# mkofinas/aether

Measured on AMD Instinct MI355X. Metric: edge-messages/sec (forward, electrostatic N=20 batch=128 per GPU), higher is better.
Workload: dtype f32; 1 GPU; electrostatic-2d-N20-B128; num_dims=2, nodes_per_graph=20, graphs_per_gpu=128, edges_per_gpu=48640, hidden=64, launch=hipgraph (10 steps per replay), parallelism=graphs sharded over 1 rank(s), no forward collective

## Files before the change

aether_amd/csrc/aether_hip.hip:

```cpp

#include <hip/hip_runtime.h>
#include <hipcub/hipcub.hpp>

#include <cstdint>
#include <cstdio>
#include <cstring>

#include "common.h"
#include "streamed.h"
#include "fused.h"
#include "backward.h"
#include "fused_bwd.h"
#include "edge_acc.h"
#include "input_grad.h"
#include "rollout_bwd.h"
#include "wide.h"
#include "seq2seq.h"
#include "s2s_filter.h"
#include "s2s_step.h"
#include "s2s_markov.h"
#include "s2s_charges.h"
#include "s2s_locs.h"
#include "s2s_dnri.h"
#include "dynfield.h"
// ... 1479 lines not shown
    if (!p || !grads || !x || !vel || !charges || !grad_field || !workspace)
        return fail(AETHER_EINVAL, "dynamic_field_backward: null pointer");
    {
        const float* const* gp = reinterpret_cast<const float* const*>(grads);
        for (size_t k = 0; k < sizeof(AetherDynFieldParams) / sizeof(const float*); ++k)
            if (!gp[k]) return fail(AETHER_EINVAL, "dynamic_field_backward: null gradient pointer");
    }
    if (num_dims != 2 && num_dims != 3) return fail(AETHER_EINVAL, "dynamic_field_backward: num_dims must be 2 or 3");
    if (n_graphs <= 0 || nodes_per_graph <= 0 || nodes_per_graph > DYNFIELD_MAX_NODES)
        return fail(AETHER_EINVAL, "dynamic_field_backward: 1..2048 nodes per graph");
    if (n_graphs >= ((int64_t)1 << 31)) return fail(AETHER_EINVAL, "dynamic_field_backward: too many graphs");
    if (workspace_bytes < aether_dynamic_field_backward_workspace_bytes(num_dims, n_graphs))
        return fail(AETHER_ESPACE, "dynamic_field_backward: workspace too small");
    hipStream_t st = (hipStream_t)stream;
    float* partial = reinterpret_cast<float*>(align_up((size_t)workspace, 256));
    if (num_dims == 2) {
        kb_dynfield<2><<<dim3((unsigned)n_graphs), dim3(256), 0, st>>>(*p, x, vel, charges, grad_field, partial, nodes_per_graph,
                                                                       grad_field_inputs);
        k_dynfield_reduce<2><<<dim3((DynOff<2>::total + 31) / 32), dim3(256), 0, st>>>(partial, n_graphs, *grads);
    } else {
        kb_dynfield<3><<<dim3((unsigned)n_graphs), dim3(256), 0, st>>>(*p, x, vel, charges, grad_field, partial, nodes_per_graph,
                                                                       grad_field_inputs);
        k_dynfield_reduce<3><<<dim3((DynOff<3>::total + 31) / 32), dim3(256), 0, st>>>(partial, n_graphs, *grads);
    }
    HIP_OK(hipGetLastError());
    return AETHER_OK;
}

int64_t aether_debug_fetch(const char* name, int num_dims, int64_t n_nodes, int64_t n_edges,
                           const void* workspace, float* dst, void* stream) {
    if (!name || !workspace || !dst) return fail(AETHER_EINVAL, "debug_fetch: null pointer");
    if (num_dims != 2 && num_dims != 3) return fail(AETHER_EINVAL, "debug_fetch: num_dims");
    const int D = num_dims, NIS = D == 2 ? 16 : 24;
    WsLayout W(n_nodes, n_edges, D, false);
    const char* ws = (const char*)workspace;
    hipStream_t st = (hipStream_t)stream;
    auto copy2d = [&](const float* src, int64_t rows, int src_ld, int col0, int cols) -> int64_t {
        hipError_t e = hipMemcpy2DAsync(dst, (size_t)cols * 4, src + col0, (size_t)src_ld * 4,
                                        (size_t)cols * 4, (size_t)rows, hipMemcpyDeviceToDevice, st);
        if (e != hipSuccess) { fail(AETHER_EHIP, hipGetErrorString(e)); return AETHER_EHIP; }
        return rows * cols;
    };
    const float* ni = (const float*)(ws + W.nodeinfo);
    if (!strcmp(name, "field")) return copy2d(ni, n_nodes, NIS, 2 * D, D);
    if (!strcmp(name, "R")) return copy2d(ni, n_nodes, NIS, 3 * D, D * D);
    if (!strcmp(name, "canon")) return copy2d(ni, n_nodes, NIS, 3 * D + D * D, 2 * D);
    if (!strcmp(name, "stamps"))
        return copy2d((const float*)(ws + W.stamps), 4096, FUSED_STAMPS, 0, FUSED_STAMPS);
    if (name[0] == 'x' && name[1] >= '0' && name[1] <= '4' && !name[2])
        return copy2d((const float*)(ws + W.x[name[1] - '0']), n_nodes, H, 0, H);
    if (name[0] == 'e' && name[1] >= '1' && name[1] <= '4' && !name[2])
        return copy2d((const float*)(ws + W.e[name[1] - '1']), n_edges, H, 0, H);
    if (!strcmp(name, "efeat"))
        return copy2d((const float*)(ws + W.feat), n_edges, FPAD, 0, FPAD);
    return fail(AETHER_EINVAL, "debug_fetch: unknown name");
}

int aether_debug_split(const float* x, int n_tiles, uint16_t* hi, uint16_t* lo, int* on, float* scale, float* y) {
    if (!x || !hi || !lo || !on || !scale || !y) return fail(AETHER_EINVAL, "debug_split: null pointer");
    if (n_tiles < 0) return fail(AETHER_EINVAL, "debug_split: n_tiles");
    if (n_tiles == 0) return AETHER_OK;
    k_debug_split<<<dim3(1), dim3(64 * DEBUG_SPLIT_WAVES), 0, nullptr>>>(x, n_tiles, hi, lo, on, scale, y);
    HIP_OK(hipGetLastError());
    return AETHER_OK;
}

int aether_s2s_launch_stats(AetherS2SLaunchStats* stats) {
    if (!stats) return fail(AETHER_EINVAL, "s2s_launch_stats: null pointer");
    *stats = g_s2s_stats;
    return AETHER_OK;
}

void aether_s2s_launch_stats_reset(void) { g_s2s_stats = AetherS2SLaunchStats{}; }

int aether_debug_fused_packed_edge(int wave, int lane) {
    if (wave < 0 || wave >= FUSED_PACK_WAVES || lane < 0 || lane >= FUSED_PACK_LANES) return -1;
    return fused_packed_edge(wave, lane);
}

int aether_debug_fused_wave_role(int what, int wave) {
    if (wave < 0 || wave >= 12) return -1;
    if (what == 0) return wave >= FUSED_FRAME_WAVE0 && fused_frame_tile(wave) < FUSED_MAX_NODES / 16 ? fused_frame_tile(wave) : -1;
    if (what == 1) return wave >= FUSED_X0_WAVE0 && fused_x0_rowblock(wave) < FUSED_X0_WAVES ? fused_x0_rowblock(wave) : -1;
    return -1;
}

#include "host_wide.inc"
#include "host_rollout_train.inc"

}
```

aether_amd/csrc/fused.h:

```cpp
#pragma once
#include "common.h"
#include "fused_layout.h"
#include "fused_graph.h"
#include "fused_handoff.h"

namespace {

struct FusedDebug {
    float* nodeinfo; float* x[5]; float* e[4];
    float* n[4]; float* ps[3]; float* pr[3]; float* feat;
    int* flags;
    int* errword;
    const float* wimg;
    float* stamps;
    StepExtras step;
};
constexpr int FUSED_STAMPS = 512;

#ifdef AETHER_FUSED_STAMPS
#define FUSED_STAMP(id)                                                                          \
    do {                                                                                         \
        if (tid == 0 && blockIdx.x < 4096)                                                       \
            dbg.stamps[blockIdx.x * FUSED_STAMPS + (id)] = (float)(wall_clock64() - t_entry) * 0.01f; \
    } while (0)
// ... 11 lines not shown
    } while (0)
#define FUSED_PSTAMP_W(w_, k_, dep_)                                                              \
    do {                                                                                         \
        asm volatile("v_mov_b32 %0, %0" : "+v"(dep_));                                           \
        if (wave == (w_) && lane == 0 && blockIdx.x < 4096)                                      \
            dbg.stamps[blockIdx.x * FUSED_STAMPS + 400 + (k_)] =                                  \
                (float)(__builtin_amdgcn_s_memtime() - c_entry);                                 \
    } while (0)
#define FUSED_PSTAMP(k_, dep_) FUSED_PSTAMP_W(0, k_, dep_)
#else
#define FUSED_STAMP(id)
#define FUSED_WSTAMP(layer_, r_, k_)
#define FUSED_WSTAMP_ROWS(layer_, r_)
#define FUSED_PSTAMP(k_, dep_)
#define FUSED_PSTAMP_W(w_, k_, dep_)
#endif

template <int D, int NW, int ROUNDS, bool KEEP, bool GRAN = false>
__global__ void __launch_bounds__(NW * 64)
k_fused(AetherParams P, const float* __restrict__ x, const float* __restrict__ vel,
        const float* __restrict__ charges, const float* __restrict__ edge_attr_orig,
        const int32_t* __restrict__ perm, const int32_t* __restrict__ send_s,
        const int32_t* __restrict__ recv_s, const int32_t* __restrict__ rowptr,
        const FusedWG* __restrict__ wgdesc, const uint32_t* __restrict__ trec, const int4* __restrict__ ledge,
        const int32_t* __restrict__ nrange, FusedDebug dbg, float* __restrict__ out) {
    constexpr bool keep = KEEP;
    using NI = NodeInfo<D>;
    using L = FusedLds<NW, ROUNDS>;
    constexpr int THREADS = NW * 64;
    constexpr int FIN = 2 * D + 16;
    static_assert(NW == 8 || NW == 12, "waves 0-7 run the node phase; NW == 12 adds four waves that run step 3 (DESIGN.md 4.1)");
    static_assert(NW == 8 || (ROUNDS == 1 && !KEEP), "the 12-wave kernel owns one tile per wave and saves nothing for the backward");
    static_assert(!GRAN || NW == 12, "granules are the 12-wave kernel's hand-off");
    constexpr bool LATE = NW == 12 || ROUNDS == 2;
    constexpr bool EARLY = NW == 12;
    extern __shared__ __attribute__((aligned(16))) float smem[];
    float* wA = smem + L::WA;
    float* wB = smem + L::WB;
    const float* cblk = smem + L::CBLK;
    float* xbuf = smem + L::XBUF;
    float* nbuf = smem + L::NBUF;
    float* psb = smem + L::PS;
    float* prb = smem + L::PR;
    float* ninfo = smem + L::NINFO;
    float* part = smem + L::PART;

    const int tid = threadIdx.x, lane = tid & 63, wave = tid >> 6;
    const int i = lane & 15, q = lane >> 4;
    const FusedWG wg = wgdesc[blockIdx.x];
    const int vb = wg.vb, nv = wg.ve - wg.vb;
    const int nb = wg.nb, ne = wg.ne;
    const int n = ne - nb, off = nb - vb;
    const int eb = wg.eb, m = wg.m;
    const int n_tiles = (m + 15) >> 4;
    const int na = wg.na;
    typedef __attribute__((address_space(3))) volatile int lds_word;
    lds_word* arrived = (lds_word*)(smem + L::ARRIVED);
    if (tid == 0) { arrived[0] = 0; arrived[1] = 0; }
#ifdef AETHER_FUSED_STAMPS
    const unsigned long long t_entry = wall_clock64();
    const unsigned long long c_entry = __builtin_amdgcn_s_memtime();
#endif
    FUSED_STAMP(0);

    auto dma_images = [&](int layer_) {
        const int na_frag = layer_ == 1 ? 8 : 16, nw_frag = na_frag + 16;
        const int total = nw_frag + FUSED_CBLK / 256;
        const int wv = __builtin_amdgcn_readfirstlane(wave);
        __builtin_assume(wv >= 0 && wv < NW);
        const int g_img = fused_wimg_offset(layer_, 0), g_cb = fused_cblk_offset(layer_);
        const int l_cb = L::CBLK + (layer_ & 1) * FUSED_CBLK;
        constexpr int MAXF = (32 + FUSED_CBLK / 256 + NW - 1) / NW;
#pragma unroll
        for (int j = 0; j < MAXF; ++j) {
            const int f = wv + NW * j;
            if (f < total) {
                const int img = f < na_frag ? f * 256 : FUSED_WIMG + (f - na_frag) * 256;
                const int soff = f < nw_frag ? g_img + img : g_cb + (f - nw_frag) * 256;
                const int doff = f < nw_frag ? L::WA + img : l_cb + (f - nw_frag) * 256;
                __builtin_amdgcn_global_load_lds(dbg.wimg + soff + lane * 4, (__attribute__((address_space(3))) void*)(smem + doff), 16, 0, 0);
            }
        }
    };
    dma_images(1);
    FUSED_STAMP(1);

    constexpr int FR = ROUNDS < 2 ? ROUNDS : 2;
    constexpr bool PACKED = NW == 12;
    constexpr bool FIMG = NW == 12;
    constexpr bool FRAMES = NW == 12;
    f32x4 x0_acc = f32x4{0.f, 0.f, 0.f, 0.f}, x0_ar = f32x4{0.f, 0.f, 0.f, 0.f};
    const int f_local = PACKED ? fused_packed_edge(wave, lane) : 16 * (NW * (lane >> 4) + wave) + (lane & 15);
    const bool f_have = (PACKED ? wave < FUSED_PACK_WAVES && lane < FUSED_PACK_LANES : lane < 16 * FR) && f_local < m;
    int4 f_e = make_int4(0, 0, 0, 0);
    f32x2 f_ea = {0.0f, 0.0f};
    int4 t_e[ROUNDS];
    unsigned seg_ends[ROUNDS];
    unsigned seg_rows[ROUNDS][4];
    {
        const int wv = __builtin_amdgcn_readfirstlane(wave);
#pragma unroll
        for (int r = 0; r < ROUNDS; ++r) {
            const int stile = NW * r + wv;
            const uint32_t* rec = trec + (size_t)(wg.tile0 + (stile < n_tiles ? stile : 0)) * FUSED_TREC;
            seg_ends[r] = stile < n_tiles ? __builtin_amdgcn_readfirstlane(rec[0]) : 0u;
#pragma unroll
            for (int w = 0; w < 4; ++w) seg_rows[r][w] = __builtin_amdgcn_readfirstlane(rec[2 + w]);
        }
    }
    const int aslot = (tid >> 4) & (FUSED_MAX_NODES - 1), ac4 = (tid & 15) * 4;
    int4 nr_rec;
    const int4* own_desc = reinterpret_cast<const int4*>(wgdesc + blockIdx.x);
    const int4* le_base = m > 0 ? ledge + eb : own_desc;
    const int4* nr_base = n > 0 ? reinterpret_cast<const int4*>(nrange) + nb : own_desc;
    const float* ea_base = m > 0 ? edge_attr_orig : reinterpret_cast<const float*>(own_desc);
    const float* qattr = dbg.step.qattr;
    auto index_stage_a = [&]() {
        f_e = le_base[f_have ? f_local : 0];
#pragma unroll
        for (int r = 0; r < ROUNDS; ++r) {
            const int tile = NW * r + wave, local = 16 * tile + i;
            t_e[r] = le_base[local < m ? local : 0];
        }
        nr_rec = nr_base[aslot < n ? aslot : 0];
    };
    auto index_select = [&]() {
        if (!f_have) f_e = make_int4(0, 0, 0, 0);
#pragma unroll
        for (int r = 0; r < ROUNDS; ++r) {
            t_e[r].x = m > 0 ? t_e[r].x : 0; t_e[r].y = m > 0 ? t_e[r].y : vb;
            t_e[r].z = m > 0 ? t_e[r].z : nb; t_e[r].w = m > 0 ? t_e[r].w : 0;
        }
    };
    auto index_stage_b = [&]() -> f32x2 {
        f32x2 v;
        if (qattr) {
            v[0] = qattr[f_e.y]; v[1] = qattr[f_e.z];
        } else {
            const float* ea = ea_base + 2 * (int64_t)f_e.w;
            v[0] = ea[0]; v[1] = ea[1];
        }
        return v;
    };

    {
        const int vtiles = (nv + 15) >> 4;
        if (wave < vtiles) {
            const float* p_ext;
            int node;
            bool live;
            int64_t g;
            float pz[D], vz[D], ef[D];
            float ch;
            float zc[6][3], a1[2][6];
            f32x4 w2f[2][2], w4f[2], acc1[2], acc2[2];
            f32x4 acc3 = f32x4{0.f, 0.f, 0.f, 0.f};
            float ar[4][2];
            f32x4 acc0[4];
            f32x4 fimg[FIMG ? FUSED_FIMG_CHUNKS : 1];
            if constexpr (FIMG) {
                const auto fimg_rsrc = __builtin_amdgcn_make_buffer_rsrc(const_cast<float*>(dbg.wimg) + fused_fimg_offset(), 0, FUSED_FIMG * 4, 0x00020000);
                p_ext = dbg.step.ext_field ? dbg.step.ext_field : x;
                asm volatile("" :: "s"(fimg_rsrc), "s"(p_ext), "s"(x), "s"(vel), "s"(charges), "s"(le_base), "s"(nr_base),
                             "s"(ea_base), "s"(qattr));
                node = 16 * wave + i;
                live = node < nv;
                g = vb + (live ? node : 0);
// ... 374 lines not shown
        arange = (unsigned)at0 | (unsigned)at1 << 8 | (unsigned)bt0 << 16 | (unsigned)bt1 << 24;
        const int deg = (nr.y - nr.x) + (nr.w - nr.z);
        adeg = (float)(deg > 1 ? deg : 1);
    }

    f16x8 wsh[2], wsl[2], wrh[2], wrl[2];
    f16x8 wf_h[4], wf_l[4];
    const auto wimg_rsrc = __builtin_amdgcn_make_buffer_rsrc(const_cast<float*>(dbg.wimg), 0, FUSED_WIMG_SPLIT * 4, 0x00020000);
    const int lane16 = lane * 16;
#pragma unroll 1
    for (int layer = 1; layer <= 4; ++layer) {
        const float* cb = cblk + (layer & 1) * FUSED_CBLK;
        const int mb2 = wave & 7;
        const int mb3 = wave & 3, tn3 = (wave >> 2) & 1;
        const bool act3 = wave < 8;
        const bool one_tile = NW == 12 ? true : n <= 16;
        const int tn4 = one_tile ? 0 : tn3;
        const int tn3s = tn4;
        const bool do3 = NW == 12 ? wave >= 8 : act3 && (one_tile ? wave >= 4 : 16 * tn3 < n);
        const bool do_s = act3 && (one_tile ? wave < 4 : true);
        const bool do_r = act3 && (one_tile ? wave >= 4 : true);
        f16x8 w3h[2], w3l[2], w4h[4], w4l[4];
        auto frag = [&](int block_bytes, int kb) -> f16x8 {
            return __builtin_bit_cast(f16x8, __builtin_amdgcn_raw_buffer_load_b128(wimg_rsrc, lane16, block_bytes + kb * 1024, 0));
        };
        auto load_frags = [&](int which, int mb, int MBN, int KBN, int kb0, int nkb, f16x8* wh, f16x8* wl) {
            if constexpr (ROUNDS == 3 && KEEP) {
                const f16x8* w = reinterpret_cast<const f16x8*>(dbg.wimg + fused_nimg_offset(layer, which)) +
                                 __builtin_amdgcn_readfirstlane(mb) * (KBN * 64);
#pragma unroll
                for (int kb = kb0; kb < kb0 + nkb; ++kb) {
                    wh[kb] = w[kb * 64 + lane];
                    wl[kb] = w[MBN * KBN * 64 + kb * 64 + lane];
                }
                return;
            }
            int lbytes = (layer - 1) * (FUSED_NIMG_LAYER * 4);
            asm volatile("" : "+s"(lbytes));
            const int blk = fused_nimg_offset(1, which) * 4 + lbytes + __builtin_amdgcn_readfirstlane(mb) * (KBN * 1024);
#pragma unroll
            for (int kb = kb0; kb < kb0 + nkb; ++kb) {
                wh[kb] = frag(blk, kb);
                wl[kb] = frag(blk + MBN * KBN * 1024, kb);
            }
        };
        auto issue_loads = [&](int part) {
            if constexpr (NW == 12) {
                const int wv = __builtin_amdgcn_readfirstlane(wave);
                int lbytes = (layer - 1) * (FUSED_NIMG_LAYER * 4);
                asm volatile("" : "+s"(lbytes));
                const bool w4 = wv >= 8;
                const int blk01 = lbytes + (w4 ? fused_nimg_offset(1, 1) * 4 + (wv & 3) * 4096 : fused_nimg_offset(1, 0) * 4 + wv * 2048);
                const int blk23 = w4 ? blk01 + 2048 : lbytes + (wv < 4 ? fused_nimg_offset(1, 2) : fused_nimg_offset(1, 3)) * 4 + (wv & 3) * 2048;
                const int lo23 = w4 ? 16 * 1024 : 8 * 1024;
                if (part == 1) {
#pragma unroll
                    for (int kb = 0; kb < 2; ++kb) {
                        wf_h[kb] = frag(blk01, kb);
                        wf_l[kb] = frag(blk01 + 16 * 1024, kb);
                    }
                }
                if (part == 3) {
#pragma unroll
                    for (int kb = 0; kb < 2; ++kb) {
                        wf_h[2 + kb] = frag(blk23, kb);
                        wf_l[2 + kb] = frag(blk23 + lo23, kb);
                    }
                }
            } else {
            if (part == 1 && act3) load_frags(0, mb2, 8, 2, 0, 2, w3h, w3l);
            if ((part == 2 || part == 3) && do3) load_frags(1, mb3, 4, 4, 2 * (part - 2), 2, w4h, w4l);
            if (part == 4 && (layer < 4 ? true : act3)) {
                if (layer == 4 || do_s) load_frags(2, mb3, 4, 2, 0, 2, wsh, wsl);
                if (layer == 4 || do_r) load_frags(3, mb3, 4, 2, 0, 2, wrh, wrl);
            }
            }
        };
        const bool xch = wg.partner >= 0 && layer > 1;
        auto front_gemm = [&](int r, f32x4 (&acc)[4], bool last, bool late_tile) {
            if (layer == 1) {
#pragma unroll
                for (int mb = 0; mb < 4; ++mb) acc[mb] = ld4(cb + CB_B1 + 16 * mb + 4 * q);
                f32x4 bop[2] = {e[r][0], e[r][1]};
                gemm_split<4, 1>(wA, bop, acc, lane);
            } else {
                f32x4 pr[4], st[4];
#pragma unroll
                for (int mb = 0; mb < 4; ++mb) {
                    pr[mb] = ld4(prb + rl[r] * LDW + 16 * mb + 4 * q);
                    st[mb] = pr[mb] + ld4(psb + sl[r] * LDW + 16 * mb + 4 * q);
                }
                if (late_tile) {
                    const bool late = 16 * (NW * r + wave) + i >= na;
#pragma unroll
                    for (int mb = 0; mb < 4; ++mb)
#pragma unroll
                        for (int c = 0; c < 4; ++c) st[mb][c] = late ? pr[mb][c] : st[mb][c];
                }
                if constexpr (LATE) {
                    if constexpr (EARLY) {
#pragma unroll
                        for (int mb = 0; mb < 4; ++mb) acc[mb] = e[r][mb] + st[mb];
                    } else {
                        f32x4 g[4];
#pragma unroll
                        for (int mb = 0; mb < 4; ++mb) g[mb] = f32x4{0.f, 0.f, 0.f, 0.f};
                        gemm_split<4, 2>(wA, e[r], g, lane);
#pragma unroll
                        for (int mb = 0; mb < 4; ++mb) acc[mb] = g[mb] + st[mb];
                    }
                } else {
#pragma unroll
                    for (int mb = 0; mb < 4; ++mb) acc[mb] = st[mb];
                    gemm_split<4, 2>(wA, e[r], acc, lane);
                }
            }
        };
        auto late_add = [&](int r, f32x4 (&acc)[4]) {
            const bool late = 16 * (NW * r + wave) + i >= na;
            f32x4 ps[4];
#pragma unroll
            for (int mb = 0; mb < 4; ++mb) ps[mb] = ld4(psb + sl[r] * LDW + 16 * mb + 4 * q);
            asm volatile("s_waitcnt lgkmcnt(0)" : "+v"(ps[0]), "+v"(ps[1]), "+v"(ps[2]), "+v"(ps[3]));
#pragma unroll
            for (int mb = 0; mb < 4; ++mb)
#pragma unroll
                for (int c = 0; c < 4; ++c) acc[mb][c] = late ? acc[mb][c] + ps[mb][c] : acc[mb][c];
        };
        auto receive_partner_rows = [&]() {
            if constexpr (GRAN) {
                FUSED_WSTAMP(layer, 0, 6);
                gran_receive(gran_rsrc(dbg.flags, wg.goff, vb, nv), layer, nv, n, off, lane, psb, arrived, dbg.errword);
                asm volatile("s_waitcnt lgkmcnt(0)" ::: "memory");
                __builtin_amdgcn_wave_barrier();
                if (lane == 0) arrived[0] = layer;
                FUSED_WSTAMP(layer, 0, 7);
                return;
            }
            if (lane == 0) {
                unsigned spins = 0;
                unsigned long long t_first = 0;
                while (__hip_atomic_load(dbg.flags + wg.partner, __ATOMIC_RELAXED, __HIP_MEMORY_SCOPE_AGENT) < layer - 1) {
                    __builtin_amdgcn_s_sleep(2);
                    if ((++spins & 1023u) == 0) {
                        const unsigned long long now = wall_clock64();
                        if (t_first == 0) t_first = now;
                        if (now - t_first <= 500000000ull) continue;
                        if (dbg.errword) __hip_atomic_store(dbg.errword, 1, __ATOMIC_RELAXED, __HIP_MEMORY_SCOPE_SYSTEM);
                        arrived[1] = 1;
                        break;
                    }
                }
            }
            __builtin_amdgcn_fence(__ATOMIC_ACQUIRE, "wavefront");
            __builtin_amdgcn_wave_barrier();
            const int np = nv - n;
            typedef unsigned int u32x4 __attribute__((ext_vector_type(4)));
            const auto rsrc = __builtin_amdgcn_make_buffer_rsrc(dbg.ps[layer - 2] + (int64_t)vb * H, 0, nv * H * 4, 0x00020000);
            FUSED_WSTAMP(layer, 0, 6);
            if constexpr (NW == 12) {
                for (int base = 0; base < np * 16; base += 256) {
                    u32x4 v[4];
                    int dst[4];
#pragma unroll
                    for (int j = 0; j < 4; ++j) {
                        const int idx = base + 64 * j + lane, idc = idx < np * 16 ? idx : 0;
                        int slot = idc >> 4;
// ... 18 lines not shown
            } else
            for (int idx = lane; idx < np * 16; idx += 64) {
                int slot = idx >> 4;
                if (slot >= off) slot += n;
                const int c = (idx & 15) * 4;
                const u32x4 v = __builtin_amdgcn_raw_buffer_load_b128(rsrc, (slot * H + c) * 4, 0, 16);
                f32x4 f;
#pragma unroll
                for (int r4 = 0; r4 < 4; ++r4) f[r4] = __uint_as_float(v[r4]);
                st4(psb + slot * LDW + c, f);
            }
            asm volatile("s_waitcnt vmcnt(0) lgkmcnt(0)" ::: "memory");
            __builtin_amdgcn_wave_barrier();
            if (lane == 0) arrived[0] = layer;
            FUSED_WSTAMP(layer, 0, 7);
        };
        auto wait_partner_rows = [&]() {
            while (__builtin_amdgcn_readfirstlane(arrived[0]) < layer) __builtin_amdgcn_s_sleep(1);
            asm volatile("" ::: "memory");
        };
        auto early_product = [&]() {
            if (n_tiles > wave) {
                f32x4 g[4];
#pragma unroll
                for (int mb = 0; mb < 4; ++mb) g[mb] = f32x4{0.f, 0.f, 0.f, 0.f};
                gemm_split_paired<4, 2>(wA, e[0], g, lane);
#pragma unroll
                for (int mb = 0; mb < 4; ++mb) e[0][mb] = g[mb];
            }
        };
        auto front_act = [&](int r, f32x4 (&acc)[4], f32x4 (&h1)[4], bool last) {
            if (last) issue_loads(1);
#pragma unroll
            for (int mb = 0; mb < 4; ++mb) h1[mb] = silu4(acc[mb]);
        };
        auto back = [&](int r, const f32x4 (&h1)[4], bool last) {
            const int tile = NW * r + wave;
            f32x4 acc2[4];
            if (last) issue_loads(2);
#pragma unroll
            for (int mb = 0; mb < 4; ++mb) acc2[mb] = ld4(cb + CB_B2 + 16 * mb + 4 * q);
            gemm_split<4, 2>(wB, h1, acc2, lane);
            if (last) issue_loads(3);
#pragma unroll
            for (int mb = 0; mb < 4; ++mb) e[r][mb] = silu4(acc2[mb]);
            if constexpr (KEEP) {
                if (ke[r] >= 0 && dbg.e[layer - 1] != nullptr) {
#pragma unroll
                    for (int mb = 0; mb < 4; ++mb)
                        st4(dbg.e[layer - 1] + (int64_t)ke[r] * H + 16 * mb + 4 * q, e[r][mb]);
                }
            }
            float* wst = smem + L::WSTAGE + wave * (16 * LDST);
#pragma unroll
            for (int mb = 0; mb < 4; ++mb) st4(wst + i * LDST + 16 * mb + 4 * q, e[r][mb]);
            FUSED_WSTAMP(layer, r, 4);
            __builtin_amdgcn_wave_barrier();
            {
                float cv[16];
#pragma unroll
                for (int k = 0; k < 16; ++k) cv[k] = wst[k * LDST + lane];
                float* pcol = part + lane;
                unsigned ends = seg_ends[r];
                asm volatile("" : "+s"(ends));
                unsigned long long lo = (unsigned long long)seg_rows[r][0] | ((unsigned long long)seg_rows[r][1] << 32);
                unsigned long long hi = (unsigned long long)seg_rows[r][2] | ((unsigned long long)seg_rows[r][3] << 32);
                float sum = 0.0f;
#pragma unroll
                for (int k = 0; k < 16; ++k) {
                    sum += cv[k];
                    if ((ends >> k) & 1u) {
                        pcol[((unsigned)lo & 0xFFu) * LDW] = sum;
                        sum = 0.0f;
                        lo = (lo >> 8) | (hi << 56);
                        hi >>= 8;
                    }
                }
            }
            __builtin_amdgcn_wave_barrier();
            if (last) issue_loads(4);
        };
        {
            const int nvalid = n_tiles > wave ? (n_tiles - wave + NW - 1) / NW : 0;
            if (nvalid == 0) {
#pragma unroll
                for (int part = 1; part < 5; ++part) issue_loads(part);
            }
            const int recv_wave = GRAN && na >= 16 ? 0 : NW - 1;
            if (xch && wave == recv_wave) receive_partner_rows();
            bool have_rows = !xch || wave == recv_wave;
#pragma unroll
            for (int r = 0; r < ROUNDS; ++r) {
                if (r < nvalid) {
                    const bool last = r == nvalid - 1;
                    const bool partner_tile = xch && 16 * (NW * r + wave + 1) > na;
                    const bool late_tile = LATE && partner_tile;
                    FUSED_WSTAMP(layer, r, 0);
                    if constexpr (!LATE) {
                        if (partner_tile && !have_rows) {
                            wait_partner_rows();
                            have_rows = true;
                        }
                    }
                    FUSED_WSTAMP(layer, r, 1);
                    f32x4 acc[4], h1[4];
                    front_gemm(r, acc, last, late_tile);
                    FUSED_WSTAMP(layer, r, 3);
                    if (late_tile) {
                        if (!have_rows) {
                            wait_partner_rows();
                            have_rows = true;
                        }
                        FUSED_WSTAMP_ROWS(layer, r);
                        late_add(r, acc);
                    }
                    front_act(r, acc, h1, last);
                    FUSED_WSTAMP(layer, r, 2);
                    back(r, h1, last);
                    FUSED_WSTAMP(layer, r, 5);
                }
            }
        }
        FUSED_STAMP(4 + 8 * (layer - 1) + 2);
        lds_barrier();
        FUSED_STAMP(4 + 8 * (layer - 1) + 3);
        if (tid < FUSED_MAX_NODES * 16) {
            f32x4 sum = f32x4{0.f, 0.f, 0.f, 0.f};
            const int at0 = arange & 0xFF, at1 = (arange >> 8) & 0xFF, bt0 = (arange >> 16) & 0xFF, bt1 = arange >> 24;
            for (int t = at0; t < at1; ++t) sum += ld4(part + (aslot + t) * LDW + ac4);
            for (int t = bt0; t < bt1; ++t) sum += ld4(part + (aslot + t) * LDW + ac4);
            const f32x4 nv = ld4(xbuf + aslot * LDW + ac4) + sum / adeg;
            st4(nbuf + aslot * LDW + ac4, nv);
            if constexpr (NW == 12) {
                if (wave < 4) {
                    pieces_store(smem + L::NPC, aslot, tid & 3, (tid & 15) >> 2, nv);
                    range_word_store(smem + L::PFLAG + wave, absmax4(0.0f, nv), lane);
                }
            }
            if (keep && aslot < n) st4(dbg.n[layer - 1] + (int64_t)(nb + aslot) * H + ac4, nv);
        }
        __builtin_amdgcn_s_waitcnt(0x0F70);
        if (layer < 4) dma_images(layer + 1);
        lds_barrier();
        FUSED_STAMP(4 + 8 * (layer - 1) + 7);
        if (act3) {
            float* ubuf = smem + L::UBUF;
            const f32x4 bv = ld4(cb + CB_B3 + 16 * mb2 + 4 * q);
#pragma unroll
            for (int tn = 0; tn < (NW == 12 ? 1 : 2); ++tn) {
                if (16 * tn < n) {
                    if constexpr (NW == 12) {
                        const f16x8 wh2[2] = {wf_h[0], wf_h[1]}, wl2[2] = {wf_l[0], wf_l[1]};
                        const f32x4 uv = silu4(gemm_pieces_regs(wh2, wl2, smem + L::NPC, smem + L::PFLAG, nbuf + i * LDW + 4 * q, lane, bv));
                        st4(ubuf + i * LDU + 16 * mb2 + 4 * q, uv);
                        pieces_store(smem + L::UPC + (mb2 >> 2) * SPLIT_PIECES, i, q, mb2 & 3, uv);
                        range_word_store(smem + L::PFLAG + 4 + mb2, absmax4(0.0f, uv), lane);
                    } else {
                        f32x4 nv[4];
#pragma unroll
                        for (int a = 0; a < 4; ++a) nv[a] = ld4(nbuf + (16 * tn + i) * LDW + 16 * a + 4 * q);
                        const f32x4 acc = gemm_split_regs<2>(w3h, w3l, nv, bv);
                        st4(ubuf + (16 * tn + i) * LDU + 16 * mb2 + 4 * q, silu4(acc));
                    }
                }
            }
        }
        if constexpr (EARLY) {
            if (layer < 4) __builtin_amdgcn_s_waitcnt(0x0F70);
        }
        lds_barrier();
        FUSED_STAMP(4 + 8 * (layer - 1) + 4);
        if constexpr (EARLY) {
            if (layer < 4 && wave < 8) {
                FUSED_WSTAMP(layer + 1, 0, 8);
                early_product();
                FUSED_WSTAMP(layer + 1, 0, 9);
            }
        }

        if (do3) {
            const float* ubuf = smem + L::UBUF;
            f32x4 acc = ld4(cb + CB_B4 + 16 * mb3 + 4 * q);
#pragma unroll
            for (int hk = 0; hk < 2; ++hk) {
                if constexpr (NW == 12) {
                    const f16x8 wh2[2] = {wf_h[2 * hk], wf_h[2 * hk + 1]}, wl2[2] = {wf_l[2 * hk], wf_l[2 * hk + 1]};
                    acc = gemm_pieces_regs(wh2, wl2, smem + L::UPC + hk * SPLIT_PIECES, smem + L::PFLAG + 4 + 4 * hk,
                                           ubuf + i * LDU + 64 * hk + 4 * q, lane, acc);
                } else {
                    f32x4 uv[4];
#pragma unroll
                    for (int a = 0; a < 4; ++a) uv[a] = ld4(ubuf + (16 * tn3s + i) * LDU + 16 * (4 * hk + a) + 4 * q);
                    const f16x8 wh2[2] = {w4h[2 * hk], w4h[2 * hk + 1]}, wl2[2] = {w4l[2 * hk], w4l[2 * hk + 1]};
                    acc = gemm_split_regs<2>(wh2, wl2, uv, acc);
                }
            }
            acc += ld4(nbuf + (16 * tn3s + i) * LDW + 16 * mb3 + 4 * q);
            st4(xbuf + (16 * tn3s + i) * LDW + 16 * mb3 + 4 * q, acc);
            if constexpr (NW == 12) {
                pieces_store(smem + L::XPC, i, q, mb3, acc);
                range_word_store(smem + L::PFLAG + 12 + mb3, absmax4(0.0f, acc), lane);
            }
            if (keep && 16 * tn3s + i < n)
                st4(dbg.x[layer] + (int64_t)(nb + 16 * tn3s + i) * H + 16 * mb3 + 4 * q, acc);
        }
        lds_barrier();
        FUSED_STAMP(4 + 8 * (layer - 1) + 5);
        if (layer < 4) {
            if constexpr (GRAN && !EARLY) __builtin_amdgcn_s_waitcnt(0x0F70);
            if constexpr (EARLY) {
                if (wave >= 8) {
                    FUSED_WSTAMP(layer + 1, 0, 8);
                    early_product();
                    FUSED_WSTAMP(layer + 1, 0, 9);
                }
            }
            if (16 * tn4 < n) {
                f32x4 xv[4];
                if constexpr (NW != 12) {
#pragma unroll
                    for (int a = 0; a < 4; ++a) xv[a] = ld4(xbuf + (16 * tn4 + i) * LDW + 16 * a + 4 * q);
                }
                if (do_s) {
                    f32x4 accs;
                    if constexpr (NW == 12) {
                        const f16x8 wh2[2] = {wf_h[2], wf_h[3]}, wl2[2] = {wf_l[2], wf_l[3]};
                        accs = gemm_pieces_regs(wh2, wl2, smem + L::XPC, smem + L::PFLAG + 12, xbuf + i * LDW + 4 * q, lane,
                                                f32x4{0.f, 0.f, 0.f, 0.f});
                    } else {
                        accs = gemm_split_regs<2>(wsh, wsl, xv, f32x4{0.f, 0.f, 0.f, 0.f});
                    }
                    if (16 * tn4 + i < n) {
                        st4(psb + (off + 16 * tn4 + i) * LDW + 16 * mb3 + 4 * q, accs);
                        float* gps = dbg.ps[layer - 1] + (int64_t)(nb + 16 * tn4 + i) * H + 16 * mb3 + 4 * q;
                        if (GRAN && wg.partner >= 0) {
                            gran_publish(gran_rsrc(dbg.flags, wg.goff, vb, nv), off + 16 * tn4 + i, 16 * mb3 + 4 * q, layer, accs);
                        } else if (wg.partner >= 0) {
                            typedef unsigned int u32x4 __attribute__((ext_vector_type(4)));
                            const auto rsrc = __builtin_amdgcn_make_buffer_rsrc(
                                dbg.ps[layer - 1] + (int64_t)nb * H, 0, n * H * 4, 0x00020000);
                            u32x4 bits;
#pragma unroll
                            for (int r4 = 0; r4 < 4; ++r4) bits[r4] = __float_as_uint(accs[r4]);
                            __builtin_amdgcn_raw_buffer_store_b128(bits, rsrc, ((16 * tn4 + i) * H + 16 * mb3 + 4 * q) * 4, 0, 16);
                        } else if (keep) {
                            st4(gps, accs);
                        }
                    }
                }
                if (do_r) {
                    f32x4 accr;
                    if constexpr (NW == 12) {
                        const f16x8 wh2[2] = {wf_h[2], wf_h[3]}, wl2[2] = {wf_l[2], wf_l[3]};
                        accr = gemm_pieces_regs(wh2, wl2, smem + L::XPC, smem + L::PFLAG + 12, xbuf + i * LDW + 4 * q, lane,
                                                ld4(cb + CB_B1N + 16 * mb3 + 4 * q));
                    } else {
                        accr = gemm_split_regs<2>(wrh, wrl, xv, ld4(cb + CB_B1N + 16 * mb3 + 4 * q));
                    }
                    st4(prb + (16 * tn4 + i) * LDW + 16 * mb3 + 4 * q, accr);
                    if (keep && 16 * tn4 + i < n)
                        st4(dbg.pr[layer - 1] + (int64_t)(nb + 16 * tn4 + i) * H + 16 * mb3 + 4 * q, accr);
                }
            }
            if (!GRAN)
                asm volatile("s_waitcnt vmcnt(0)" ::: "memory");
            lds_barrier();
            if (!GRAN && wg.partner >= 0 && tid == 0)
                __hip_atomic_store(dbg.flags + blockIdx.x, layer, __ATOMIC_RELAXED, __HIP_MEMORY_SCOPE_AGENT);
            FUSED_STAMP(4 + 8 * (layer - 1) + 6);
        }
    }
    if (wg.partner >= 0 && tid == 0)
        __hip_atomic_store(dbg.flags + wg.partner, 0, __ATOMIC_RELAXED, __HIP_MEMORY_SCOPE_AGENT);
    if constexpr (GRAN) {
        if (wg.partner >= 0 && wave >= 8) gran_rearm(gran_rsrc(dbg.flags, wg.goff, vb, nv), nv, n, off, tid - 512, 256);
    }

    {
        float* o1 = smem + L::OBUF1;
        float* o2 = smem + L::OBUF2;
        const int mb = wave & 3, tn = NW == 12 ? 0 : (wave >> 2) & 1;
        const bool act = wave < 8 && 16 * tn < n;
        const bool act1 = NW == 12 ? wave < 4 && n > 0 : act;
        const bool act2 = NW == 12 ? wave >= 4 && wave < 8 && n > 0 : act;
        const float* cb = cblk;
        if (act1) {
            f32x4 acc;
            if constexpr (NW == 12) {
                const f16x8 wh2[2] = {wf_h[2], wf_h[3]}, wl2[2] = {wf_l[2], wf_l[3]};
                acc = gemm_pieces_regs(wh2, wl2, smem + L::XPC, smem + L::PFLAG + 12, xbuf + i * LDW + 4 * q, lane,
                                       ld4(cb + CB_B1N + 16 * mb + 4 * q));
            } else {
                f32x4 xv[4];
#pragma unroll
// ... 77 lines not shown
```

aether_amd/csrc/fused_layout.h:

```cpp
#pragma once
#include "common.h"

namespace {

constexpr int FUSED_MAX_NODES = 32;
constexpr int FUSED_MAX_EDGES = 384;
constexpr int FUSED_MAX_TILES = FUSED_MAX_EDGES / 16;
constexpr int LDU = 2 * H + 8;
constexpr int FUSED_PACK_WAVES = 4, FUSED_PACK_LANES = 48;
__device__ __host__ constexpr int fused_packed_edge(int wave, int lane) { return FUSED_PACK_LANES * wave + lane; }
static_assert(FUSED_PACK_WAVES * FUSED_PACK_LANES == 12 * 16 && FUSED_PACK_LANES % 16 == 0, "every row of the twelve tiles has one builder");
constexpr int FUSED_FRAME_WAVE0 = 2, FUSED_X0_WAVE0 = 4, FUSED_X0_WAVES = 4;
__device__ __host__ constexpr int fused_frame_tile(int wave) { return wave - FUSED_FRAME_WAVE0; }
__device__ __host__ constexpr int fused_x0_rowblock(int wave) { return wave - FUSED_X0_WAVE0; }
static_assert(FUSED_FRAME_WAVE0 >= FUSED_MAX_NODES / 16 && FUSED_FRAME_WAVE0 + FUSED_MAX_NODES / 16 <= 12 && FUSED_X0_WAVE0 + FUSED_X0_WAVES <= 12 &&
              FUSED_X0_WAVES * 16 == H, "frame waves behind the field waves, one x0 wave per 16 of the H rows");

constexpr int FUSED_WIMG = SPLIT_WIMG;
constexpr int FUSED_CBLK = 768;
constexpr int CB_B1 = 0;
constexpr int CB_B2 = 64;
constexpr int CB_B3 = 128;
constexpr int CB_B4 = 256;
constexpr int CB_B1N = 320;
constexpr int CB_OB3 = 384;
constexpr int CB_OB6 = 448;
constexpr int CB_OW6 = 512;
template <int NW, int ROUNDS> struct FusedLds {
    static constexpr int WSZ = FUSED_WIMG;
    static constexpr int WA = 0;
    static constexpr int WB = WA + WSZ;
    static constexpr int CBLK = WB + WSZ;
    static constexpr int XBUF = CBLK + 2 * FUSED_CBLK;
    static constexpr int NBUF = XBUF + FUSED_MAX_NODES * LDW;
    static constexpr int PS = NBUF + FUSED_MAX_NODES * LDW;
    static constexpr int PR = PS + FUSED_MAX_NODES * LDW;
    static constexpr int NINFO = PR + FUSED_MAX_NODES * LDW;
    static constexpr int PART_ROWS = ROUNDS == 3 ? FUSED_MAX_NODES + FUSED_MAX_TILES : 2 * FUSED_MAX_NODES + 16;
    static constexpr int PART = NINFO + FUSED_MAX_NODES * 24;
    static constexpr int ARRIVED = PART + PART_ROWS * LDW;
    static constexpr int SCRATCH = ARRIVED + 4;
    static constexpr int FEAT_ROWS = 16 * (ROUNDS < 2 ? ROUNDS : 2);
    static constexpr int SCRATCH_SIZE =
        NW * FEAT_ROWS * LDF > NW * 16 * LDST ? NW * FEAT_ROWS * LDF : NW * 16 * LDST;
    static constexpr int TOTAL = SCRATCH + SCRATCH_SIZE;
    static constexpr int FIELD_Z = SCRATCH;
    static constexpr int FIELD_H1 = FIELD_Z + FUSED_MAX_NODES * 24;
    static constexpr int FIELD_H2 = FIELD_H1 + FUSED_MAX_NODES * 32;
    static constexpr int FIELD_F = FIELD_H2 + FUSED_MAX_NODES * 32;
    static constexpr int FIELD_W = FIELD_F + FUSED_MAX_NODES * 4;
    static constexpr int FW0 = FIELD_W;
    static constexpr int FW2 = FW0 + 32 * 22;
    static constexpr int FW4 = FW2 + 32 * 32;
    static constexpr int FB = FW4 + 3 * 32;
    static constexpr int FEMB = FB + 68;
    static constexpr int FIELD_END = FEMB + 48;
    static constexpr int FEAT = SCRATCH;
    static constexpr int WSTAGE = SCRATCH;
    static constexpr int UBUF = SCRATCH;
    static constexpr int OBUF1 = SCRATCH;
    static constexpr int OBUF2 = SCRATCH + FUSED_MAX_NODES * LDW;
    static constexpr int NPC = SCRATCH + (LDU > 2 * LDW ? LDU : 2 * LDW) * FUSED_MAX_NODES;
    static constexpr int UPC = NPC + SPLIT_PIECES;
    static constexpr int XPC = UPC + 2 * SPLIT_PIECES;
    static constexpr int OPC = XPC + SPLIT_PIECES;
    static constexpr int PFLAG = OPC + SPLIT_PIECES;
    static_assert(NW != 12 || (NPC >= OBUF2 + FUSED_MAX_NODES * LDW && NPC >= UBUF + FUSED_MAX_NODES * LDU && PFLAG + 5 * 4 <= TOTAL && NPC % 4 == 0), "operand pieces");
    static_assert(FIELD_END <= TOTAL, "field scratch");
    static_assert(UBUF + FUSED_MAX_NODES * LDU <= TOTAL, "ubuf");
    static_assert(OBUF2 + FUSED_MAX_NODES * LDW <= TOTAL, "obuf");
    static_assert(TOTAL * 4 <= 160 * 1024, "LDS budget");
};

constexpr int FUSED_NIMG_W3 = 2 * 8 * 2 * 64 * 4, FUSED_NIMG_W4 = 2 * 4 * 4 * 64 * 4, FUSED_NIMG_WS = 2 * 4 * 2 * 64 * 4;
constexpr int FUSED_NIMG_LAYER = FUSED_NIMG_W3 + FUSED_NIMG_W4 + 2 * FUSED_NIMG_WS;
constexpr int FI_ACC1 = 0;
constexpr int FI_ACC2 = 8;
constexpr int FI_W2F = 16;
constexpr int FI_W4F = 32;
constexpr int FI_ACC3 = 40;
constexpr int FI_ACC0 = 44;
constexpr int FI_A1 = 60;
constexpr int FI_ZC = 72;
constexpr int FI_AR = 90;
constexpr int FI_END = 98;
constexpr int FUSED_FIMG_CHUNKS = (FI_END + 3) / 4;
static_assert(FI_ACC0 % 4 == 0 && FI_AR % 4 == 2, "an x0 wave's operands: one whole chunk and half of another");
__device__ __host__ constexpr bool fused_fimg_x0_slot(int s) { return (s >= FI_ACC0 && s < FI_A1) || (s >= FI_AR && s < FI_END); }
__device__ __host__ constexpr bool fused_fimg_field_chunk(int c) {
    for (int r = 0; r < 4; ++r)
        if (4 * c + r < FI_END && !fused_fimg_x0_slot(4 * c + r)) return true;
    return false;
}
constexpr int FUSED_FIMG = FUSED_FIMG_CHUNKS * 256;
constexpr int FUSED_WIMG_SPLIT = 8 * FUSED_WIMG + 4 * FUSED_NIMG_LAYER + 4 * FUSED_CBLK;
constexpr int FUSED_WIMG_SET = FUSED_WIMG_SPLIT + FUSED_FIMG;
constexpr int FUSED_SPLIT_BLOCKS = 8 + 4 * 6 + 1 + FUSED_FIMG_CHUNKS;
__device__ __host__ constexpr int fused_fimg_offset() { return FUSED_WIMG_SPLIT; }
__device__ __host__ constexpr int fused_wimg_offset(int layer, int which) { return ((layer - 1) * 2 + which) * FUSED_WIMG; }
__device__ __host__ constexpr int fused_nimg_offset(int layer, int which) {
    return 8 * FUSED_WIMG + (layer - 1) * FUSED_NIMG_LAYER +
           (which == 0 ? 0 : which == 1 ? FUSED_NIMG_W3 : which == 2 ? FUSED_NIMG_W3 + FUSED_NIMG_W4 : FUSED_NIMG_W3 + FUSED_NIMG_W4 + FUSED_NIMG_WS);
}
__device__ __host__ constexpr int fused_cblk_offset(int layer) { return 8 * FUSED_WIMG + 4 * FUSED_NIMG_LAYER + (layer - 1) * FUSED_CBLK; }

__device__ __forceinline__ float fused_cblk_value(const AetherParams& P, int nd, int layer, int c) {
    if (c < CB_B2) return layer == 1 ? P.l1_msg_b0[c] : 0.0f;
    if (c < CB_B3) return (layer == 1 ? P.l1_msg_b2 : P.ln_msg_b2[layer - 2])[c - CB_B2];
    if (c < CB_B4) return (layer == 1 ? P.l1_upd_b0 : P.ln_upd_b0[layer - 2])[c - CB_B3];
    if (c < CB_B1N) return (layer == 1 ? P.l1_upd_b2 : P.ln_upd_b2[layer - 2])[c - CB_B4];
    if (c < CB_OB3) return (layer < 4 ? P.ln_msg_b0[layer - 1] : P.out_b0)[c - CB_B1N];
    if (layer < 4) return 0.0f;
    if (c < CB_OB6) return P.out_b3[c - CB_OB3];
    if (c < CB_OB6 + 4) return c - CB_OB6 < nd ? P.out_b6[c - CB_OB6] : 0.0f;
    if (c >= CB_OW6 && c < CB_OW6 + nd * H) return P.out_w6[c - CB_OW6];
    return 0.0f;
}

__device__ __forceinline__ float fused_fimg_value(const AetherParams& P, int nd, int slot, int i, int q) {
    const int fin = 2 * nd + 16;
    if (slot < FI_ACC2) return P.field_b0[16 * (slot >> 2) + 4 * q + (slot & 3)];
    if (slot < FI_W2F) return P.field_b2[16 * ((slot - FI_ACC2) >> 2) + 4 * q + (slot & 3)];
    if (slot < FI_W4F) {
        const int s = slot - FI_W2F, mb = s >> 3, a = (s >> 2) & 1;
        return P.field_w2[(16 * mb + i) * 32 + 16 * a + 4 * q + (s & 3)];
    }
    if (slot < FI_ACC3) {
        const int s = slot - FI_W4F;
        return i < nd ? P.field_w4[i * 32 + 16 * (s >> 2) + 4 * q + (s & 3)] : 0.0f;
    }
    if (slot < FI_ACC0) return 4 * q + (slot - FI_ACC3) < nd ? P.field_b4[4 * q + (slot - FI_ACC3)] : 0.0f;
    if (slot < FI_A1) return P.l1_res_b[16 * ((slot - FI_ACC0) >> 2) + 4 * q + (slot & 3)];
    if (slot < FI_ZC) {
        const int s = slot - FI_A1, mb = s / 6, k = 4 * (s % 6) + q;
        return k < fin ? P.field_w0[(16 * mb + i) * fin + k] : 0.0f;
    }
    if (slot < FI_AR) {
        const int s = slot - FI_ZC, c = s % 3, k = 4 * (s / 3) + q;
        return (k >= 2 * nd && k < fin) ? P.field_emb[c * 16 + k - 2 * nd] : 0.0f;
    }
    if (slot < FI_END) {
        const int s = slot - FI_AR, mb = s >> 1, k = 4 * (s & 1) + q;
        return k < 2 * nd ? P.l1_res_w[(16 * mb + i) * 3 * nd + nd + k] : 0.0f;
    }
    return 0.0f;
}

__device__ __forceinline__ void split_weights_block(const AetherParams& P, int f1, int nd, float* __restrict__ wimg, int block, int tid) {
    if (block >= FUSED_SPLIT_BLOCKS - FUSED_FIMG_CHUNKS) {
// ... 62 lines not shown
```

Baseline: 6.664 billion edge-messages/s.

## Prefetch next layer's weight images earlier and split DMA across idle waves

```diff
diff --git a/aether_amd/csrc/aether_hip.hip b/aether_amd/csrc/aether_hip.hip
--- a/aether_amd/csrc/aether_hip.hip
+++ b/aether_amd/csrc/aether_hip.hip
@@ -1585,6 +1585,8 @@
     if (wave < 0 || wave >= 12) return -1;
     if (what == 0) return wave >= FUSED_FRAME_WAVE0 && fused_frame_tile(wave) < FUSED_MAX_NODES / 16 ? fused_frame_tile(wave) : -1;
     if (what == 1) return wave >= FUSED_X0_WAVE0 && fused_x0_rowblock(wave) < FUSED_X0_WAVES ? fused_x0_rowblock(wave) : -1;
+    if (what == 3) return fused_product_step(wave);
+    if (what == 4) return wave == 0 ? (FUSED_WIMG / 2) * 4 : wave == 1 ? FUSED_MAX_NODES * LDW * 4 : -1;
     return -1;
 }
 
diff --git a/aether_amd/csrc/fused.h b/aether_amd/csrc/fused.h
--- a/aether_amd/csrc/fused.h
+++ b/aether_amd/csrc/fused.h
@@ -117,7 +117,46 @@
             }
         }
     };
-    dma_images(1);
+    auto dma_frag = [&](int soff, int doff) {
+        const float* src = dbg.wimg + soff + lane * 4;
+        const unsigned dst = (unsigned)(uintptr_t)(__attribute__((address_space(3))) void*)(smem + doff);
+        asm volatile("s_mov_b32 m0, %1\n\ts_nop 0\n\tglobal_load_lds_dwordx4 %0, off" :: "v"(src), "s"(dst) : "memory", "m0");
+    };
+    auto dma_ahead = [&](int layer_, int slot, int nslots) {
+        const int g_img = fused_wimg_offset(layer_, 0), g_cb = fused_cblk_offset(layer_);
+        const int l_cb = L::CBLK + (layer_ & 1) * FUSED_CBLK;
+        constexpr int total = 16 + FUSED_CBLK / 256;
+#pragma unroll
+        for (int j = 0; j < (total + NW - 2) / (NW - 1); ++j) {
+            const int f = slot + nslots * j;
+            if (slot >= 0 && f < total) dma_frag(f < 16 ? g_img + f * 256 : g_cb + (f - 16) * 256, f < 16 ? L::WA + f * 256 : l_cb + (f - 16) * 256);
+        }
+    };
+    auto dma_w2 = [&](int layer_, int slot) {
+        const int g_img = fused_wimg_offset(layer_, 1);
+        constexpr int nw2 = NW > FUSED_W2DMA_WAVE0 ? NW - FUSED_W2DMA_WAVE0 : 1;
+        static_assert(16 % nw2 == 0, "every wave of step 2's idle ones issues the same number of fragments");
+#pragma unroll
+        for (int j = 0; j < 16 / nw2; ++j) {
+            const int f = slot + nw2 * j;
+            dma_frag(g_img + f * 256, L::WB + f * 256);
+        }
+    };
+    if constexpr (EARLY) {
+        const int wv = __builtin_amdgcn_readfirstlane(wave);
+        __builtin_assume(wv >= 0 && wv < NW);
+        constexpr int total = 8 + 16 + FUSED_CBLK / 256;
+#pragma unroll
+        for (int j = 0; j < (total + NW - 1) / NW; ++j) {
+            const int f = wv + NW * j;
+            if (f < total)
+                dma_frag(f < 8 ? fused_wimg_offset(1, 0) + f * 256 : f < 24 ? fused_wimg_offset(1, 1) + (f - 8) * 256 : fused_cblk_offset(1) + (f - 24) * 256,
+                         f < 8 ? L::W1A + f * 256 : f < 24 ? L::WB + (f - 8) * 256 : L::CBLK + FUSED_CBLK + (f - 24) * 256);
+        }
+        dma_ahead(2, wv, NW);
+    } else {
+        dma_images(1);
+    }
     FUSED_STAMP(1);
 
     constexpr int FR = ROUNDS < 2 ? ROUNDS : 2;
@@ -658,7 +697,7 @@
 #pragma unroll
                 for (int mb = 0; mb < 4; ++mb) acc[mb] = ld4(cb + CB_B1 + 16 * mb + 4 * q);
                 f32x4 bop[2] = {e[r][0], e[r][1]};
-                gemm_split<4, 1>(wA, bop, acc, lane);
+                gemm_split<4, 1>(EARLY ? smem + L::W1A : wA, bop, acc, lane);
             } else {
                 f32x4 pr[4], st[4];
 #pragma unroll
@@ -843,6 +882,14 @@
         };
         {
             const int nvalid = n_tiles > wave ? (n_tiles - wave + NW - 1) / NW : 0;
+            if constexpr (EARLY) {
+                if (layer == 2 || layer == 3) {
+                    const int recv_wave = GRAN && na >= 16 ? 0 : NW - 1;
+                    const int wv = __builtin_amdgcn_readfirstlane(wave);
+                    dma_ahead(layer + 1, wv == recv_wave ? -1 : wv - (wv > recv_wave ? 1 : 0), NW - 1);
+                    __builtin_amdgcn_sched_barrier(0);
+                }
+            }
             if (nvalid == 0) {
 #pragma unroll
                 for (int part = 1; part < 5; ++part) issue_loads(part);
@@ -883,6 +930,7 @@
             }
         }
         FUSED_STAMP(4 + 8 * (layer - 1) + 2);
+        if constexpr (EARLY) __builtin_amdgcn_s_waitcnt(0x0F78);
         lds_barrier();
         FUSED_STAMP(4 + 8 * (layer - 1) + 3);
         if (tid < FUSED_MAX_NODES * 16) {
@@ -901,9 +949,14 @@
             if (keep && aslot < n) st4(dbg.n[layer - 1] + (int64_t)(nb + aslot) * H + ac4, nv);
         }
         __builtin_amdgcn_s_waitcnt(0x0F70);
-        if (layer < 4) dma_images(layer + 1);
+        if constexpr (!EARLY) {
+            if (layer < 4) dma_images(layer + 1);
+        }
         lds_barrier();
         FUSED_STAMP(4 + 8 * (layer - 1) + 7);
+        if constexpr (EARLY) {
+            if (layer < 4 && wave >= FUSED_W2DMA_WAVE0) dma_w2(layer + 1, __builtin_amdgcn_readfirstlane(wave) - FUSED_W2DMA_WAVE0);
+        }
         if (act3) {
             float* ubuf = smem + L::UBUF;
             const f32x4 bv = ld4(cb + CB_B3 + 16 * mb2 + 4 * q);
@@ -926,13 +979,10 @@
                 }
             }
         }
-        if constexpr (EARLY) {
-            if (layer < 4) __builtin_amdgcn_s_waitcnt(0x0F70);
-        }
         lds_barrier();
         FUSED_STAMP(4 + 8 * (layer - 1) + 4);
         if constexpr (EARLY) {
-            if (layer < 4 && wave < 8) {
+            if (layer < 4 && fused_product_step(wave) == 3) {
                 FUSED_WSTAMP(layer + 1, 0, 8);
                 early_product();
                 FUSED_WSTAMP(layer + 1, 0, 9);
@@ -968,9 +1018,9 @@
         lds_barrier();
         FUSED_STAMP(4 + 8 * (layer - 1) + 5);
         if (layer < 4) {
-            if constexpr (GRAN && !EARLY) __builtin_amdgcn_s_waitcnt(0x0F70);
+            if constexpr (GRAN) __builtin_amdgcn_s_waitcnt(0x0F70);
             if constexpr (EARLY) {
-                if (wave >= 8) {
+                if (fused_product_step(wave) == 4) {
                     FUSED_WSTAMP(layer + 1, 0, 8);
                     early_product();
                     FUSED_WSTAMP(layer + 1, 0, 9);
diff --git a/aether_amd/csrc/fused_layout.h b/aether_amd/csrc/fused_layout.h
--- a/aether_amd/csrc/fused_layout.h
+++ b/aether_amd/csrc/fused_layout.h
@@ -15,6 +15,10 @@
 __device__ __host__ constexpr int fused_x0_rowblock(int wave) { return wave - FUSED_X0_WAVE0; }
 static_assert(FUSED_FRAME_WAVE0 >= FUSED_MAX_NODES / 16 && FUSED_FRAME_WAVE0 + FUSED_MAX_NODES / 16 <= 12 && FUSED_X0_WAVE0 + FUSED_X0_WAVES <= 12 &&
               FUSED_X0_WAVES * 16 == H, "frame waves behind the field waves, one x0 wave per 16 of the H rows");
+
+constexpr int FUSED_STEP3_WAVE0 = 8;
+__device__ __host__ constexpr int fused_product_step(int wave) { return wave < FUSED_STEP3_WAVE0 ? 3 : 4; }
+constexpr int FUSED_W2DMA_WAVE0 = FUSED_STEP3_WAVE0;
 
 constexpr int FUSED_WIMG = SPLIT_WIMG;
 constexpr int FUSED_CBLK = 768;
@@ -65,6 +69,8 @@
     static constexpr int XPC = UPC + 2 * SPLIT_PIECES;
     static constexpr int OPC = XPC + SPLIT_PIECES;
     static constexpr int PFLAG = OPC + SPLIT_PIECES;
+    static constexpr int W1A = PS;
+    static_assert(FUSED_WIMG / 2 <= FUSED_MAX_NODES * LDW && W1A % 256 == 0, "layer 1's image A fits the P_s rows, on a fragment boundary");
     static_assert(NW != 12 || (NPC >= OBUF2 + FUSED_MAX_NODES * LDW && NPC >= UBUF + FUSED_MAX_NODES * LDU && PFLAG + 5 * 4 <= TOTAL && NPC % 4 == 0), "operand pieces");
     static_assert(FIELD_END <= TOTAL, "field scratch");
     static_assert(UBUF + FUSED_MAX_NODES * LDU <= TOTAL, "ubuf");
```

Result: faster. 6.778 billion edge-messages/s, median of 6 (+1.7%).
